# sssxyd/cpp-paddle-ocr

Hardware: AMD Instinct MI355X
Metric: images/sec end-to-end (det+cls+rec) at 960x960 (higher is better)
Workload: dtype f32

## Files before the change

cpp-paddle-ocr_amd/binding.py:

```python
import ctypes as C
import os

import numpy as np

HERE = os.path.dirname(os.path.abspath(__file__))
ROOT = os.path.dirname(HERE)
LIB_PATH = os.environ.get("OCR_LIB_PATH") or os.path.join(HERE, "lib", "libocr_hip.so")
MODELS = os.path.join(ROOT, "models")

_lib = None


class OcrError(RuntimeError):
    pass


class ocr_img(C.Structure):
    _fields_ = [("data", C.c_void_p), ("rows", C.c_int), ("cols", C.c_int), ("row_stride", C.c_size_t)]


class ocr_det_cfg(C.Structure):
    _fields_ = [("model_dir", C.c_char_p), ("device_id", C.c_int), ("limit_type", C.c_char_p),
                ("limit_side_len", C.c_int), ("det_db_thresh", C.c_double), ("det_db_box_thresh", C.c_double),
                ("det_db_unclip_ratio", C.c_double), ("det_db_score_mode", C.c_char_p), ("use_dilation", C.c_int),
# ... 800 lines not shown
class ocr_char(C.Structure):
    _fields_ = [("step", C.c_int32), ("nsteps", C.c_int32), ("prob", C.c_float), ("quad", C.c_int32 * 8)]


EXPORTS += ["ocr_pipe_cfg_default", "ocr_pipe_create", "ocr_pipe_destroy", "ocr_pipe_run", "ocr_pipe_run_chars", "ocr_pipe_run_device",
            "ocr_pipe_stage", "ocr_pipe_slot_probs", "ocr_pipe_run_staged", "ocr_pipe_run_device_on", "ocr_pipe_run_staged_on", "ocr_pipe_stage_jpeg", "ocr_jpeg_decode", "ocr_jpeg_time",
            "ocr_pipe_stage_jpeg_frames", "ocr_jpeg_decode_frame", "ocr_jpeg_time_frame", "ocr_pipe_slot_image",
            "ocr_png_decode", "ocr_png_time", "ocr_png_time_batch", "ocr_pipe_stage_coded",
            "ocr_raw_decode", "ocr_raw_time", "ocr_raw_time_batch", "ocr_pipe_stage_frames",
            "ocr_tiff_decode", "ocr_tiff_time", "ocr_tiff_time_batch", "ocr_pipe_stage_batch",
            "ocr_webp_decode", "ocr_webp_time", "ocr_webp_time_batch", "ocr_vp8_decode", "ocr_vp8_time", "ocr_vp8_time_batch", "ocr_j2k_decode", "ocr_j2k_time", "ocr_j2k_time_batch",
            "ocr_j2k_tier1", "ocr_j2k_decode_coded", "ocr_j2k_time_coded", "ocr_j2k_time_coded_batch",
            "ocr_tiff_expand", "ocr_tiff_decode_coded", "ocr_tiff_time_coded", "ocr_tiff_time_coded_batch",
            "ocr_tiff_inflate", "ocr_tiff_decode_deflate", "ocr_tiff_time_deflate", "ocr_tiff_time_deflate_batch",
            "ocr_pipe_label", "ocr_pipe_det_shape", "ocr_pipe_stats", "ocr_pipe_timing", "ocr_pipe_timing_filter", "ocr_pipe_timing_report", "ocr_dev_alloc",
            "ocr_dev_free", "ocr_dev_upload", "ocr_dev_download", "ocr_dev_sync", "ocr_dev_copy_time", "ocr_rotate_crop", "ocr_rotate_crop_shape", "ocr_rotate180_rois"]


def _pipe_protos(L):
    if getattr(L, "_pipe_protos_done", False):
        return
    _stage_protos(L)
    vp, ip = C.c_void_p, C.POINTER(C.c_int)
    L.ocr_pipe_cfg_default.argtypes = [C.POINTER(ocr_pipe_cfg)]
    L.ocr_pipe_create.argtypes = [C.POINTER(ocr_pipe_cfg), C.POINTER(vp)]
    L.ocr_pipe_destroy.argtypes = [vp]
    L.ocr_pipe_run.argtypes = [vp, C.POINTER(ocr_img), C.c_int, vp, C.c_int, vp, vp, vp, C.c_int, C.POINTER(C.c_double)]
    L.ocr_pipe_run_chars.argtypes = [vp, C.POINTER(ocr_img), C.c_int, vp, C.c_int, vp, vp, vp, C.c_int, vp, C.POINTER(C.c_double)]
    L.ocr_pipe_run_device.argtypes = [vp, vp, C.c_int, C.c_int, C.c_int, vp, vp, C.c_int, vp, vp, vp, C.c_int,
                                      C.POINTER(C.c_double)]
    L.ocr_pipe_stage.argtypes = [vp, C.c_int, C.POINTER(ocr_img), C.c_int]
# ... 473 lines not shown
            maps = [np.ascontiguousarray(p, dtype=np.float32) for p in probs]
            for i, m in enumerate(maps):
                arr[i] = m.ctypes.data
            check(lib().ocr_pipe_slot_probs(self.h, slot, arr, n))

    def stage_dev_probs(self, slot, imgs, dev_probs):
        n = len(imgs)
        self._staged_n = getattr(self, "_staged_n", {})
        check(lib().ocr_pipe_stage(self.h, slot, _imgs(imgs), n))
        self._staged_n[slot] = n
        arr = (C.c_void_p * n)()
        for i, d in enumerate(dev_probs):
            arr[i] = d.ptr.value
        check(lib().ocr_pipe_slot_probs(self.h, slot, arr, n))

    def stats(self):
        out = (C.c_longlong * 3)()
        check(lib().ocr_pipe_stats(self.h, out))
        return dict(runs=int(out[0]), binds=int(out[1]), graph_replays=int(out[2]))

    def run_staged(self, slot, collect=True):
        count = self._staged_n[slot]
        words, ids = self._bufs(count)
        off = np.zeros(count, np.int32)
        nw = np.zeros(count, np.int32)
        check(lib().ocr_pipe_run_staged(self.h, slot, words, self._cap_words, off.ctypes.data, nw.ctypes.data, ids.ctypes.data,
                                        self._cap_ids, self.times))
        return self._collect(count, words, ids, off, nw) if collect else int(nw.sum())

    def run_device(self, dev_imgs, rows, cols, count, dev_prob=None, collect=True):
# ... 67 lines not shown
```

cpp-paddle-ocr_amd/csrc/capi_net.hip:

```cpp
#include <cstdio>
#include <atomic>
#include <cstring>
#include <mutex>
#include <vector>

#include "capi_common.h"
#include "plans_embedded.inc"

__attribute__((constructor)) static void ocr_runtime_env_defaults() { setenv("GPU_MAX_HW_QUEUES", "16", 0); }

namespace ocr {

const RtOptions& rt_options() {
  static RtOptions o;
  static std::once_flag once;
  std::call_once(once, [] {
    auto off = [](const char* n) { const char* e = getenv(n); return e && e[0] == '0'; };
    auto num = [](const char* n, long def) { const char* e = getenv(n); return e && *e ? atol(e) : def; };
    o.fuse = !off("OCR_FUSE");
    o.fuse_gap_min = num("OCR_FUSE_GAP_MIN", 64 * 1024);
    o.conv_small_nt = !off("OCR_CONV_SMALL_NT");
    o.conv_mt2 = !off("OCR_CONV_MT2");
    if (const char* e = getenv("OCR_CONV_MT2")) o.conv_mt2_force = e[0] == 'f';
    o.conv_c24 = !off("OCR_CONV_C24");
    { const char* e = getenv("OCR_DW_LDS"); o.dw_lds = !(e && e[0] == '0'); }
    { const char* e = getenv("OCR_DWPW2"); o.dwpw2 = !(e && e[0] == '0'); }
    { const char* e = getenv("OCR_XDW"); o.xdw = !(e && e[0] == '0'); }
    { const char* e = getenv("OCR_MFMA_X16"); o.mfma_x16 = !(e && e[0] == '0'); }
    { const char* e = getenv("OCR_ATTN_LINE"); o.attn_line = !(e && e[0] == '0'); }
    o.dwpw_items = (int)num("OCR_DWPW_ITEMS", 32);
    o.dwpw_force_upw = (int)num("OCR_DWPW_FORCE_UPW", 0);
    if (const char* e = getenv("OCR_DWPW_T4")) o.dwpw_t4_thin = e[0] == 't';
    o.trace_slice = (int)num("OCR_TRACE_SLICE", 0);
  });
  return o;
}
static std::mutex g_refuse_mu;
static std::string g_refuse;
static std::atomic<bool> g_refuse_on{false};
std::string rt_refuse_launch() {
  if (!g_refuse_on.load(std::memory_order_acquire)) return std::string();
  std::lock_guard<std::mutex> lk(g_refuse_mu);
  return g_refuse;
}
void rt_set_refuse_launch(const char* substr) {
  std::lock_guard<std::mutex> lk(g_refuse_mu);
  g_refuse = substr ? substr : "";
  g_refuse_on.store(!g_refuse.empty(), std::memory_order_release);
// ... 417 lines not shown
```

cpp-paddle-ocr_amd/csrc/pipe.hip:

```cpp
#include <algorithm>
#include <array>
#include <chrono>
#include <cstring>
#include <functional>
#include <map>
#include <memory>
#include <thread>

#include "capi_common.h"
#include "crop.h"
#include "frame_kinds.h"
#include "stages.h"

using namespace ocr;

namespace {
double now_ms() {
  return std::chrono::duration<double, std::milli>(std::chrono::steady_clock::now().time_since_epoch()).count();
}
}

using CharLists = std::vector<std::vector<ocr_char>>;
static int emit(const std::vector<std::vector<ocr_word>>& W, const std::vector<std::vector<int32_t>>& I, const std::vector<int>& order,
                ocr_word* words, int cap_words, int* word_off, int* nwords, int32_t* ids, int cap_ids, const CharLists* C = nullptr,
// ... 87 lines not shown
    return OCR_OK;
  }

  bool timing_on = false;
  std::string timing_filter;
  int add_det_extra(std::string& err) {
    std::unique_ptr<DetStage> d(new DetStage());
    int code = 0;
    if (!d->create(det_cfg, err, code)) return code ? code : OCR_ERR_DEVICE;
    d->net().set_timing_filter(timing_filter);
    d->net().enable_timing(timing_on);
    det_extra.push_back(std::move(d));
    return OCR_OK;
  }

  int run_images(uint8_t* base, const std::vector<StageSlot::Img>& imgs, const std::vector<StageSlot::Group>& groups, const float* probs,
                 std::vector<std::vector<ocr_word>>& out_words, std::vector<std::vector<int32_t>>& out_ids, double times[3], std::string& err,
                 CharLists* out_chars = nullptr) {
    const int count = (int)imgs.size();
    boxes.resize((size_t)count * kCap * 8);
    nbox.assign(count, 0);
    double t0 = now_ms();
    auto run_group = [&](DetStage& d, const StageSlot::Group& g, std::string& e) {
      const size_t row = (size_t)g.cols * 3, img_bytes = row * g.rows;
      return d.run_device(base + g.off, img_bytes, row, g.rows, g.cols, g.count, boxes.data() + (size_t)g.first * kCap * 8, kCap,
                          nbox.data() + g.first, nullptr, e, probs ? probs + g.prob_off : nullptr);
    };
    const int lanes = (int)std::min<size_t>((size_t)det_lanes, groups.size());
    if (groups.size() > 1 && det_ragged) {
      std::vector<DetStage::MixedGroup> mg(groups.size());
      std::vector<size_t> gpx(groups.size());
      for (size_t gi = 0; gi < groups.size(); ++gi) {
        const auto& g = groups[gi];
// ... 62 lines not shown
        for (int l = 0; l < np; ++l)
          if (rcs[l]) { err = errs[l]; return rcs[l]; }
        if (g_stream_sync(src.stream()) != hipSuccess) { err = "det stream sync failed"; return OCR_ERR_DEVICE; }
        src.collect_timings();
      }
    } else if (lanes <= 1) {
      for (const auto& g : groups) {
        int rc = run_group(det, g, err);
        if (rc) return rc;
      }
    } else {
      while ((int)det_extra.size() < lanes - 1) {
        int rc = add_det_extra(err);
        if (rc) return rc;
      }
      if (g_stream_sync(det.stream()) != hipSuccess) { err = "det stream sync failed"; return OCR_ERR_DEVICE; }
      std::vector<int> rcs(lanes, OCR_OK);
      std::vector<std::string> errs(lanes);
      auto lane_fn = [&](int l) {
        DetStage& d = l == 0 ? det : *det_extra[l - 1];
        for (size_t gi = l; gi < groups.size(); gi += lanes) {
          rcs[l] = run_group(d, groups[gi], errs[l]);
          if (rcs[l]) return;
        }
      };
      std::vector<std::thread> th;
      for (int l = 1; l < lanes; ++l) th.emplace_back(lane_fn, l);
      lane_fn(0);
      for (auto& t : th) t.join();
      for (int l = 0; l < lanes; ++l)
        if (rcs[l]) { err = errs[l]; return rcs[l]; }
// ... 25 lines not shown
          lines.push_back(LineSrc{base + imgs[i].off, row, ix0, iy0, ix1 - ix0, iy1 - iy0});
        }
      }
      seg.push_back((int)lines.size());
    }
    out_words.assign(count, {});
    out_ids.assign(count, {});
    if (out_chars) out_chars->assign(count, {});
    if (lines.empty()) return OCR_OK;
    std::vector<int> labels;
    if (cls) {
      labels.resize(lines.size());
      std::vector<float> scores(lines.size());
      int rc = cls->run_lines(lines, labels.data(), scores.data(), err);
      if (rc) return rc;
      std::vector<RotDesc> rd;
      for (size_t k = 0; k < lines.size(); ++k)
        if (labels[k] == 1) rd.push_back(RotDesc{const_cast<uint8_t*>(lines[k].img), lines[k].stride, lines[k].x, lines[k].y, lines[k].w, lines[k].h});
      int rrc = rotate180_in_order(rd, rot_desc, rot_seg, cls->stream(), err);
      if (rrc) return rrc;
      if (g_stream_sync(cls->stream()) != hipSuccess) { err = "cls stream sync failed"; return OCR_ERR_DEVICE; }
    }
    double t2 = now_ms();
    times[1] += t2 - t1;
    const int max_len = 256;
    std::vector<int32_t> ids(lines.size() * max_len);
    std::vector<int> lens(lines.size());
    std::vector<float> scores(lines.size());
    std::vector<int32_t> csteps, cnsteps, geom;
    std::vector<float> cprobs;
    int rc;
    if (out_chars) {
      csteps.resize(ids.size()); cnsteps.resize(ids.size()); cprobs.resize(ids.size()); geom.resize(lines.size() * 3);
      RecStage::CharOut co;
      co.steps = csteps.data(); co.nsteps = cnsteps.data(); co.probs = cprobs.data(); co.geom = geom.data();
      rc = rec.run_lines_chars(lines, seg, ids.data(), max_len, lens.data(), scores.data(), co, err);
// ... 11 lines not shown
        w.confidence = scores[k];
        out_ids[i].insert(out_ids[i].end(), ids.begin() + (size_t)k * max_len, ids.begin() + (size_t)k * max_len + lens[k]);
        out_words[i].push_back(w);
        if (out_chars)
          for (int j = 0; j < lens[k]; ++j) {
            const size_t q = (size_t)k * max_len + j;
            ocr_char ch;
            ch.step = csteps[q]; ch.nsteps = cnsteps[q]; ch.prob = cprobs[q];
            const LineSrc& L = lines[k];
            char_quad(ch.step, ch.nsteps, geom[3 * k], geom[3 * k + 1], geom[3 * k + 2], L.w, L.h, !labels.empty() && labels[k] == 1,
                      crop_mode == OCR_CROP_ROTATE ? &line_plan[k] : nullptr, L.x, L.y, imgs[i].rows, imgs[i].cols, ch.quad);
            (*out_chars)[i].push_back(ch);
          }
      }
    }
    return OCR_OK;
  }

  int rotate_crops(const uint8_t* base, const std::vector<StageSlot::Img>& imgs, std::vector<LineSrc>& lines, std::vector<int>& seg,
                   std::vector<int>& line_box, std::string& err) {
    std::vector<WarpDesc> wd;
    std::vector<size_t> off;
    size_t total = 0;
    int max_px = 0;
    for (int i = 0; i < (int)imgs.size(); ++i) {
      const int rows = imgs[i].rows, cols = imgs[i].cols;
      const size_t row = (size_t)cols * 3;
      for (int j = 0; j < nbox[i]; ++j) {
        CropPlan p;
        if (!plan_rotate_crop(rows, cols, &boxes[((size_t)i * kCap + j) * 8], p)) continue;
// ... 25 lines not shown
    if (g_stream_sync(det.stream()) != hipSuccess) { err = "crop kernel failed"; return OCR_ERR_DEVICE; }
    return OCR_OK;
  }
};

struct ocr_pipe {
  PipeWorker w0;
  std::vector<std::unique_ptr<PipeWorker>> extra;
  int phases = 2;
  int parts_per_chain = 1;
  int device = 0;
  StageSlot slots[2];
  hipStream_t copy_stream = nullptr;
  FrameScratch frame_scratch;
  DevBuf<uint8_t> work;
  DevBuf<uint8_t> work_chain[4];
  PipeWorker* worker(int c) { return c == 0 ? &w0 : (c >= 1 && c <= (int)extra.size() ? extra[c - 1].get() : nullptr); }

  ~ocr_pipe() { if (copy_stream) (void)hipStreamDestroy(copy_stream); }

  int layout(StageSlot& S, int count, const std::function<void(int, int&, int&)>& size_of, std::string& err) {
    if (!copy_stream && hipStreamCreateWithFlags(&copy_stream, hipStreamNonBlocking) != hipSuccess) { err = "hipStreamCreate failed"; return OCR_ERR_DEVICE; }
    if (!S.ready && hipEventCreateWithFlags(&S.ready, hipEventDisableTiming) != hipSuccess) { err = "hipEventCreate failed"; return OCR_ERR_DEVICE; }
    if (S.staged && hipEventSynchronize(S.ready) != hipSuccess) { err = "staging event failed"; return OCR_ERR_DEVICE; }
    S.staged = false;
    std::vector<int> order(count), rows(count), cols(count);
    for (int i = 0; i < count; ++i) { order[i] = i; size_of(i, rows[i], cols[i]); }
    std::stable_sort(order.begin(), order.end(), [&](int a, int b) { return rows[a] != rows[b] ? rows[a] < rows[b] : cols[a] < cols[b]; });
    const std::vector<StageSlot::Img> before = S.imgs;
    S.imgs.clear();
// ... 72 lines not shown
    if (!S.staged || count != (int)S.imgs.size()) { err = "stage the slot's images first (same count)"; return OCR_ERR_ARG; }
    if (!S.probs.ensure(S.prob_floats + 64, err)) return OCR_ERR_DEVICE;
    for (int k = 0; k < count; ++k) {
      const size_t n = (k + 1 < count ? S.imgs[k + 1].prob_off : S.prob_floats) - S.imgs[k].prob_off;
      const hipError_t e = hipMemcpyAsync(S.probs.p + S.imgs[k].prob_off, probs[S.imgs[k].orig], n * sizeof(float), hipMemcpyDefault, copy_stream);
      if (e != hipSuccess) {
        err = std::string("probability map upload failed: ") + hipGetErrorString(e);
        return OCR_ERR_DEVICE;
      }
    }
    if (hipEventRecord(S.ready, copy_stream) != hipSuccess) { err = "hipEventRecord failed"; return OCR_ERR_DEVICE; }
    S.has_probs = true;
    return OCR_OK;
  }

  int run_images(uint8_t* base, const std::vector<StageSlot::Img>& imgs, const std::vector<StageSlot::Group>& groups, const float* probs,
                 std::vector<std::vector<ocr_word>>& out_words, std::vector<std::vector<int32_t>>& out_ids, double times[3], std::string& err,
                 CharLists* out_chars = nullptr) {
    const int count = (int)imgs.size();
    const int nchains = (int)std::min<size_t>(1 + extra.size(), (size_t)count);
    if (nchains < 2) return w0.run_images(base, imgs, groups, probs, out_words, out_ids, times, err, out_chars);
    const int K = (int)std::min<size_t>((size_t)nchains * parts_per_chain, (size_t)count);
    std::vector<std::vector<StageSlot::Img>> pi(K);
    std::vector<std::vector<StageSlot::Group>> pg(K);
    std::vector<std::vector<int>> gidx(K);
    std::vector<size_t> load(K, 0);
    auto give = [&](int p, const StageSlot::Group& g, int first, int n) {
      int rh = 0, rw = 0;
      { float a, b; DetStage::resize_shape(g.rows, g.cols, w0.det.cfg().limit_type, w0.det.cfg().limit_side_len, rh, rw, a, b); }
      StageSlot::Group ng = g;
      ng.first = (int)pi[p].size();
      ng.count = n;
      ng.off = g.off + (size_t)first * g.rows * g.cols * 3;
      ng.prob_off = g.prob_off + (size_t)first * rh * rw;
      pg[p].push_back(ng);
      for (int k = 0; k < n; ++k) { pi[p].push_back(imgs[g.first + first + k]); gidx[p].push_back(g.first + first + k); }
// ... 3 lines not shown
    for (const auto& g : groups) total += (size_t)g.count * g.rows * g.cols;
    const size_t share = (total + K - 1) / K;
    for (const auto& g : groups) {
      const size_t px = (size_t)g.rows * g.cols;
      int first = 0;
      while (first < g.count) {
        const int p = (int)(std::min_element(load.begin(), load.end()) - load.begin());
        const int left = g.count - first;
        const size_t room = share > load[p] ? share - load[p] : 0;
        int n = left;
        if ((size_t)left * px > room + px / 2) n = (int)std::min<size_t>(left, std::max<size_t>(1, (room + px / 2) / px));
        give(p, g, first, n);
        first += n;
      }
    }
    if (g_stream_sync(w0.det.stream()) != hipSuccess) { err = "det stream sync failed"; return OCR_ERR_DEVICE; }
    std::vector<std::vector<std::vector<ocr_word>>> W(K);
    std::vector<std::vector<std::vector<int32_t>>> I(K);
    std::vector<CharLists> Ch(K);
    std::vector<std::array<double, 3>> t(K, std::array<double, 3>{0, 0, 0});
    std::vector<int> rc(K, OCR_OK);
    std::vector<std::string> errs(K);
    auto chain = [&](int c) {
      PipeWorker& w = c == 0 ? w0 : *extra[c - 1];
      for (int p = c; p < K; p += nchains) {
        if (pi[p].empty()) continue;
        rc[p] = w.run_images(base, pi[p], pg[p], probs, W[p], I[p], t[p].data(), errs[p], out_chars ? &Ch[p] : nullptr);
        if (rc[p]) return;
      }
    };
    std::vector<std::thread> th;
    for (int c = 1; c < nchains; ++c) th.emplace_back([&, c]() { (void)rt_set_device(device); chain(c); });
    chain(0);
    for (auto& x : th) x.join();
    for (int p = 0; p < K; ++p)
      if (rc[p]) { err = errs[p]; return rc[p]; }
    out_words.assign(count, {});
    out_ids.assign(count, {});
    if (out_chars) out_chars->assign(count, {});
    for (int p = 0; p < K; ++p)
      for (size_t k = 0; k < gidx[p].size(); ++k) {
        out_words[gidx[p][k]] = std::move(W[p][k]);
// ... 11 lines not shown
    }
    return OCR_OK;
  }

  int run_slot(int si, ocr_word* words, int cap_words, int* word_off, int* nwords, int32_t* ids, int cap_ids, double times[3], int chain = -1,
               ocr_char* chars = nullptr) {
    StageSlot& S = slots[si];
    if (!S.staged || S.imgs.empty()) return fail(OCR_ERR_ARG, "nothing staged in this slot");
    std::string err;
    PipeWorker* one = chain >= 0 ? worker(chain) : nullptr;
    if (chain >= 0 && !one) return fail(OCR_ERR_ARG, "no such chain (0 <= chain < phases)");
    PipeWorker& first = one ? *one : w0;
    DevBuf<uint8_t>& clone = one ? work_chain[chain] : work;
    if (hipStreamWaitEvent(first.det.stream(), S.ready, 0) != hipSuccess) return fail(OCR_ERR_DEVICE, "hipStreamWaitEvent failed");
    if (!clone.ensure(S.bytes + 256, err)) return fail(OCR_ERR_DEVICE, err);
    if (hipMemcpyAsync(clone.p, S.dev.p, S.bytes, hipMemcpyDeviceToDevice, first.det.stream()) != hipSuccess) return fail(OCR_ERR_DEVICE, "clone failed");
    double t[3] = {0, 0, 0};
    std::vector<std::vector<ocr_word>> W;
    std::vector<std::vector<int32_t>> I;
    CharLists C;
    CharLists* pc = chars ? &C : nullptr;
    const int rc = one ? one->run_images(clone.p, S.imgs, S.groups, S.has_probs ? S.probs.p : nullptr, W, I, t, err, pc)
                       : run_images(clone.p, S.imgs, S.groups, S.has_probs ? S.probs.p : nullptr, W, I, t, err, pc);
    if (rc) return fail(rc, err);
    if (times) { times[0] = t[0]; times[1] = t[1]; times[2] = t[2]; }
    const int count = (int)S.imgs.size();
    std::vector<int> order(count);
    for (int k = 0; k < count; ++k) order[S.imgs[k].orig] = k;
    return emit(W, I, order, words, cap_words, word_off, nwords, ids, cap_ids, pc, chars);
  }
};

static int emit(const std::vector<std::vector<ocr_word>>& W, const std::vector<std::vector<int32_t>>& I, const std::vector<int>& order,
                ocr_word* words, int cap_words, int* word_off, int* nwords, int32_t* ids, int cap_ids, const CharLists* C, ocr_char* chars) {
  int wo = 0, io = 0;
  for (size_t i = 0; i < order.size(); ++i) {
    const auto& w = W[order[i]];
    const auto& d = I[order[i]];
// ... 80 lines not shown
static int pipe_run_device(ocr_pipe* h, int chain, const void* dev_bgr, int rows, int cols, int count, const float* dev_prob, ocr_word* words,
                           int cap_words, int* word_off, int* nwords, int32_t* ids, int cap_ids, double times[3]) {
  if (!h || !dev_bgr || rows <= 0 || cols <= 0 || count < 1 || !words || !word_off || !nwords || !ids)
    return fail(OCR_ERR_ARG, "bad argument");
  CAPI_HIP(rt_set_device(h->device));
  PipeWorker* one = chain >= 0 ? h->worker(chain) : nullptr;
  if (chain >= 0 && !one) return fail(OCR_ERR_ARG, "no such chain (0 <= chain < phases)");
  PipeWorker& first = one ? *one : h->w0;
  DevBuf<uint8_t>& clone = one ? h->work_chain[chain] : h->work;
  double t[3] = {0, 0, 0};
  std::vector<std::vector<ocr_word>> W;
  std::vector<std::vector<int32_t>> I;
  std::string err;
  const size_t img_bytes = (size_t)rows * cols * 3, bytes = img_bytes * count;
  if (!clone.ensure(bytes + 256, err)) return fail(OCR_ERR_DEVICE, err);
  CAPI_HIP(hipMemcpyAsync(clone.p, dev_bgr, bytes, hipMemcpyDeviceToDevice, first.det.stream()));
  std::vector<StageSlot::Img> imgs(count);
  for (int i = 0; i < count; ++i) imgs[i] = {rows, cols, i, img_bytes * i, 0};
  const std::vector<StageSlot::Group> groups = {{rows, cols, 0, count, 0, 0}};
  const int rc = one ? one->run_images(clone.p, imgs, groups, dev_prob, W, I, t, err) : h->run_images(clone.p, imgs, groups, dev_prob, W, I, t, err);
  if (rc) return fail(rc, err);
  if (times) { times[0] = t[0]; times[1] = t[1]; times[2] = t[2]; }
  std::vector<int> order(count);
  for (int i = 0; i < count; ++i) order[i] = i;
  return emit(W, I, order, words, cap_words, word_off, nwords, ids, cap_ids);
}
int ocr_pipe_run_device(ocr_pipe* h, const void* dev_bgr, int rows, int cols, int count, const float* dev_prob, ocr_word* words,
                        int cap_words, int* word_off, int* nwords, int32_t* ids, int cap_ids, double times[3]) {
  return pipe_run_device(h, -1, dev_bgr, rows, cols, count, dev_prob, words, cap_words, word_off, nwords, ids, cap_ids, times);
}
int ocr_pipe_run_device_on(ocr_pipe* h, int chain, const void* dev_bgr, int rows, int cols, int count, const float* dev_prob,
                           ocr_word* words, int cap_words, int* word_off, int* nwords, int32_t* ids, int cap_ids, double times[3]) {
  if (chain < 0) return fail(OCR_ERR_ARG, "no such chain (0 <= chain < phases)");
  return pipe_run_device(h, chain, dev_bgr, rows, cols, count, dev_prob, words, cap_words, word_off, nwords, ids, cap_ids, times);
}
// ... 290 lines not shown
  DevBuf<int> dseg;
  if (!dimg.ensure(row * rows, err)) return fail(OCR_ERR_DEVICE, err);
  std::vector<RotDesc> rd(n);
  for (int k = 0; k < n; ++k) {
    const int32_t* r = rects + 4 * k;
    if (r[0] < 0 || r[1] < 0 || r[2] < 1 || r[3] < 1 || r[0] + r[2] > cols || r[1] + r[3] > rows) return fail(OCR_ERR_ARG, "rectangle outside the image");
    rd[k] = RotDesc{dimg.p, row, r[0], r[1], r[2], r[3]};
  }
  CAPI_HIP(g_memcpy2d(dimg.p, row, bgr, stride, row, rows, hipMemcpyHostToDevice));
  const int rc = rotate180_in_order(rd, ddesc, dseg, 0, err);
  if (rc) return fail(rc, err);
  CAPI_HIP(g_memcpy2d(bgr, stride, dimg.p, row, row, rows, hipMemcpyDeviceToHost));
  return OCR_OK;
}

int ocr_dev_alloc(void** p, size_t bytes) {
  if (!p) return fail(OCR_ERR_ARG, "null argument");
  CAPI_HIP(g_malloc(p, bytes));
  return OCR_OK;
}
int ocr_dev_free(void* p) { CAPI_HIP(g_free(p)); return OCR_OK; }
int ocr_dev_upload(void* dst, const void* src, size_t bytes) { CAPI_HIP(g_memcpy(dst, src, bytes, hipMemcpyHostToDevice)); return OCR_OK; }
int ocr_dev_download(void* dst, const void* src, size_t bytes) { CAPI_HIP(g_memcpy(dst, src, bytes, hipMemcpyDeviceToHost)); return OCR_OK; }
int ocr_dev_sync(void) { CAPI_HIP(hipDeviceSynchronize()); return OCR_OK; }

}
```

cpp-paddle-ocr_amd/csrc/rt_options.h:

```cpp
#pragma once
#include <string>

namespace ocr {

struct RtOptions {
  bool fuse = true;
  long fuse_gap_min = 65536;
  bool conv_small_nt = true;
  bool conv_mt2 = true;
  bool conv_mt2_force = false;
  bool conv_c24 = true;
  bool attn_line = true;
  bool mfma_x16 = true;
  bool dw_lds = true;
  bool xdw = true;
  bool dwpw2 = true;
  int dwpw_items = 32;
  int dwpw_force_upw = 0;
  bool dwpw_t4_thin = false;
  int trace_slice = 0;
};
const RtOptions& rt_options();

std::string rt_refuse_launch();
void rt_set_refuse_launch(const char* substr);

}
```

cpp-paddle-ocr_amd/csrc/stages.h:

```cpp
#pragma once
#include <hip/hip_runtime.h>

#include <memory>
#include <string>
#include <vector>

#include "../../include/ocr_hip.h"
#include "kernels_post.h"
#include "kernels_pre.h"
#include "net.h"
#include "srv_net.h"

namespace ocr {

template <class T>
struct DevBuf {
  T* p = nullptr;
  size_t cap = 0;
  ~DevBuf() { if (p) (void)g_free(p); }
  bool ensure(size_t n, std::string& err) {
    if (n <= cap) return true;
    if (p) (void)g_free(p);
    p = nullptr;
    cap = 0;
// ... 116 lines not shown
                float* scores, std::string& err, const CharOut* co = nullptr);
  int run_chars(const ocr_img* imgs, int n, int32_t* ids, int max_len, int* lens, float* scores, const CharOut& co, double times[3],
                std::string& err);
  int run_lines_chars(const std::vector<LineSrc>& lines, const std::vector<int>& seg, int32_t* ids, int max_len, int* lens,
                      float* scores, const CharOut& co, std::string& err) {
    return run_lines(lines, seg, ids, max_len, lens, scores, err, &co);
  }
  int logits_row(int index, int step, float* out, size_t cap_floats, std::string& err);
  bool want_taps = true;
  int max_lines_per_launch = 4096;
  const std::vector<std::string>& labels() const { return labels_; }
  hipStream_t stream() const { return stream_; }
  Net& net() { return net_; }
  SrvNet* srv() { return srv_.get(); }
  std::vector<int> tap_T, tap_off;
  std::vector<int> tap_amax;
  std::vector<float> tap_pmax;

 private:
  RecConfig cfg_;
  Net net_;
  std::unique_ptr<SrvNet> srv_;
  hipStream_t stream_ = nullptr;
  StageTimer timer_;
  std::vector<std::string> labels_;
  DevBuf<float> lut_, pmax_, scores_, x_;
  DevBuf<int> amax_, ids_, lens_;
  DevBuf<uint8_t> staging_;
  DevBuf<LineDesc> descs_;
  DevBuf<int> csteps_, cnsteps_, alt_ids_;
// ... 42 lines not shown
```

cpp-paddle-ocr_amd/csrc/stages.hip:

```cpp
#include "stages.h"

#include <algorithm>
#include <array>
#include <cmath>
#include <cstring>
#include <fstream>
#include <map>

#include "capi_common.h"

namespace ocr {

#define ST_HIP(expr)                                                              \
  do {                                                                            \
    hipError_t _e = (expr);                                                       \
    if (_e != hipSuccess) {                                                       \
      err = std::string(#expr) + ": " + hipGetErrorString(_e);                    \
      return OCR_ERR_DEVICE;                                                      \
    }                                                                             \
  } while (0)

bool StageTimer::init(std::string& err) {
  for (int i = 0; i < 4; ++i)
    if (hipEventCreate(&ev[i]) != hipSuccess) { err = "hipEventCreate failed"; return false; }
// ... 673 lines not shown
  auto mobile_logits = [&](Net::HeadLogits& hl, const Slot& sl, bool ragged) -> int {
    if (topk <= 0) return OCR_OK;
    if (!net_.head_logits(hl, err)) return OCR_ERR_DEVICE;
    if (hl.C != C) { err = "dictionary size does not match the CTC head"; return OCR_ERR_MODEL; }
    if (ragged)
      for (int j = 0; j < sl.count; ++j)
        if ((int)hl.row0.size() != sl.count + 1 || hl.row0[j] != d[sl.first + j].step0) { err = "ragged logits rows do not match the step table"; return OCR_ERR_DEVICE; }
    return OCR_OK;
  };
  ST_HIP(hipMemcpyAsync(descs_.p, d.data(), (size_t)ni * sizeof(LineDesc), hipMemcpyHostToDevice, stream_));
  for (Slot& sl : slots) {
    if (!srv_) net_.set_head_outputs(nullptr, amax_.p + sl.step_off, pmax_.p + sl.step_off);
    if (srv_) {
      const int Wt = items[sl.first].tensor_w;
      launch_line_pre(descs_.p + sl.first, sl.count, imgH, Wt, lut_.p, false, x_.p, stream_);
      if (!srv_->run(x_.p, sl.count, imgH, Wt, stream_, err)) return OCR_ERR_DEVICE;
      const SrvTensor& ot = srv_->tensor(srv_->output_tid());
      if (ot.h != 1) { err = "rec_img_h does not reduce to a single row"; return OCR_ERR_ARG; }
      if (ot.c != (int)labels_.size()) { err = "dictionary size does not match the CTC head"; return OCR_ERR_MODEL; }
      sl.T = ot.w;
      if (sl.T > Wt / 4 + 8) { err = "rec step buffer too small"; return OCR_ERR_CAPACITY; }
      if (srv_->ctc_partials())
        srv::launch_ctc_reduce((const float*)srv_->tensor_ptr(srv_->output_tid()), (long)sl.count * sl.T, srv_->ctc_slots(), srv_->ctc_step(),
                               amax_.p + sl.step_off, pmax_.p + sl.step_off, stream_);
      else
        srv::launch_argmax_softmax((const float*)srv_->tensor_ptr(srv_->output_tid()), (long)sl.count * sl.T, ot.c, ot.cs, amax_.p + sl.step_off,
                                   pmax_.p + sl.step_off, srv_->half(), stream_);
      if (co) {
        const int rc = collapse(sl, nullptr, sl.T, (const float*)srv_->tensor_ptr(srv_->output_tid()), ot.cs);
        if (rc) return rc;
      } else
      launch_ctc(amax_.p + sl.step_off, pmax_.p + sl.step_off, sl.count, sl.T, max_len, ids_.p + (size_t)sl.first * max_len,
                 lens_.p + sl.first, scores_.p + sl.first, stream_);
    } else if (sl.ragged) {
      widths.resize(sl.count);
      long pix = 0;
      for (int j = 0; j < sl.count; ++j) { widths[j] = items[sl.first + j].tensor_w; pix += (long)imgH * widths[j]; }
      launch_line_pre_ragged(descs_.p + sl.first, sl.count, pix, imgH, lut_.p, x_.p, stream_);
      if (!net_.run_ragged(x_.p, imgH, widths.data(), sl.count, stream_, err)) return OCR_ERR_DEVICE;
      if (co) {
        Net::HeadLogits hl;
        int rc = mobile_logits(hl, sl, true);
        if (!rc) rc = collapse(sl, descs_.p + sl.first, 0, hl.ptr, hl.pitch);
        if (rc) return rc;
      } else
      launch_ctc_ragged(amax_.p + sl.step_off, pmax_.p + sl.step_off, descs_.p + sl.first, sl.count, max_len,
                        ids_.p + (size_t)sl.first * max_len, lens_.p + sl.first, scores_.p + sl.first, stream_);
    } else {
      const int Wt = items[sl.first].tensor_w;
      launch_line_pre(descs_.p + sl.first, sl.count, imgH, Wt, lut_.p, false, x_.p, stream_);
      if (!net_.run(x_.p, sl.count, imgH, Wt, stream_, err)) return OCR_ERR_DEVICE;
      const TensorDesc& ot = net_.tensor(net_.output_tid());
      if (ot.h != 1) { err = "rec_img_h does not reduce to a single row"; return OCR_ERR_ARG; }
      if (ot.c != (int)labels_.size()) { err = "dictionary size does not match the CTC head"; return OCR_ERR_MODEL; }
      sl.T = ot.w;
      if (sl.T > Wt / 4 + 8) { err = "rec step buffer too small"; return OCR_ERR_CAPACITY; }
      if (co) {
        Net::HeadLogits hl;
        int rc = mobile_logits(hl, sl, false);
        if (!rc) rc = collapse(sl, nullptr, sl.T, hl.ptr, hl.pitch);
        if (rc) return rc;
      } else
      launch_ctc(amax_.p + sl.step_off, pmax_.p + sl.step_off, sl.count, sl.T, max_len, ids_.p + (size_t)sl.first * max_len,
                 lens_.p + sl.first, scores_.p + sl.first, stream_);
    }
// ... 131 lines not shown
```

include/ocr_hip.h:

```cpp
#ifndef OCR_HIP_H_
#define OCR_HIP_H_

#include <stddef.h>
#include <stdint.h>

#ifdef __cplusplus
extern "C" {
#endif

#define OCR_OK 0
#define OCR_ERR_ARG (-1)
#define OCR_ERR_MODEL (-2)
#define OCR_ERR_DEVICE (-3)
#define OCR_ERR_CAPACITY (-4)

const char* ocr_last_error(void);
int ocr_rt_init(int device_id);
int ocr_rt_device_count(void);
int ocr_rt_set_wait_mode(int mode);
int ocr_rt_get_wait_mode(void);

typedef struct ocr_img {
  const uint8_t* data;
  int rows, cols;
// ... 325 lines not shown
} ocr_coded_frame;
int ocr_pipe_stage_batch(ocr_pipe* h, int slot, const ocr_coded_frame* frames, int count);
const char* ocr_pipe_label(ocr_pipe* h, int id);
int ocr_pipe_det_shape(ocr_pipe* h, int rows, int cols, int* net_rows, int* net_cols);
int ocr_pipe_stats(ocr_pipe* h, long long out[3]);
int ocr_pipe_timing(ocr_pipe* h, int enable);
int ocr_pipe_timing_filter(ocr_pipe* h, const char* substr);
int ocr_pipe_timing_report(ocr_pipe* h, char* buf, size_t cap);

int ocr_rotate_crop(const uint8_t* bgr, int rows, int cols, size_t row_stride, const int32_t* boxes, int n, uint8_t* out,
                    size_t out_cap, size_t* out_off, int* out_rows, int* out_cols);
int ocr_rotate_crop_shape(int rows, int cols, const int32_t* box, int* out_rows, int* out_cols);

int ocr_rotate180_rois(uint8_t* bgr, int rows, int cols, size_t row_stride, const int32_t* rects, int n);

int ocr_dev_alloc(void** p, size_t bytes);
int ocr_dev_free(void* p);
int ocr_dev_upload(void* dst, const void* src, size_t bytes);
int ocr_dev_download(void* dst, const void* src, size_t bytes);
int ocr_dev_sync(void);
int ocr_dev_copy_time(void* dst, const void* src, size_t bytes, int iters, double* ms);

typedef struct ocr_net ocr_net;
int ocr_net_create(const char* kind, const char* model_dir, const char* weights, int device_id, ocr_net** out);
int ocr_net_create_precision(const char* kind, const char* model_dir, const char* weights, int device_id, const char* precision,
                             ocr_net** out);
void ocr_net_destroy(ocr_net* h);
int ocr_net_forward(ocr_net* h, const float* x, int N, int H, int W, int keep_all);
int ocr_net_forward_ragged(ocr_net* h, const float* x, int N, int H, const int* widths, int keep_all);
int ocr_net_forward_ragged_images(ocr_net* h, const float* x, int N, const int* heights, const int* widths, int keep_all);
// ... 75 lines not shown
```

Measured before the change: 1234.

## Clone staged images lazily, only those whose crops the classifier rotates

Stops copying the whole staged image batch into a work buffer before detection. Only images that contain a line classified as upside-down are copied, with adjacent images merged into one copy, and their lines are redirected to the copy before the in-place 180-degree rotation. The source buffer is no longer modified. When lazy cloning is on, the det stream sync before the lanes is skipped because no clone copy has to finish, and the cls stream sync is skipped when nothing is rotated. The risk is an ordering hazard between the reduced syncs and the det and rec streams. A self-test entry point and a flag to turn the behaviour off are also added.

```diff
diff --git a/cpp-paddle-ocr_amd/binding.py b/cpp-paddle-ocr_amd/binding.py
--- a/cpp-paddle-ocr_amd/binding.py
+++ b/cpp-paddle-ocr_amd/binding.py
@@ -838,7 +838,8 @@
             "ocr_tiff_expand", "ocr_tiff_decode_coded", "ocr_tiff_time_coded", "ocr_tiff_time_coded_batch",
             "ocr_tiff_inflate", "ocr_tiff_decode_deflate", "ocr_tiff_time_deflate", "ocr_tiff_time_deflate_batch",
             "ocr_pipe_label", "ocr_pipe_det_shape", "ocr_pipe_stats", "ocr_pipe_timing", "ocr_pipe_timing_filter", "ocr_pipe_timing_report", "ocr_dev_alloc",
-            "ocr_dev_free", "ocr_dev_upload", "ocr_dev_download", "ocr_dev_sync", "ocr_dev_copy_time", "ocr_rotate_crop", "ocr_rotate_crop_shape", "ocr_rotate180_rois"]
+            "ocr_dev_free", "ocr_dev_upload", "ocr_dev_download", "ocr_dev_sync", "ocr_dev_copy_time", "ocr_rotate_crop", "ocr_rotate_crop_shape", "ocr_rotate180_rois",
+            "ocr_selftest_pipe_lazy_clone", "ocr_selftest_pipe_turns"]
 
 
 def _pipe_protos(L):
@@ -1342,6 +1343,30 @@
             arr[i] = d.ptr.value
         check(lib().ocr_pipe_slot_probs(self.h, slot, arr, n))
 
+    def set_lazy_clone(self, on):
+        L = lib()
+        L.ocr_selftest_pipe_lazy_clone.argtypes = [C.c_void_p, C.c_int]
+        check(L.ocr_selftest_pipe_lazy_clone(self.h, int(bool(on))))
+
+    def selftest_turns(self, imgs, rects, labels, owner):
+        imgs = np.ascontiguousarray(imgs, dtype=np.uint8)
+        assert imgs.ndim == 4 and imgs.shape[3] == 3
+        rects = np.ascontiguousarray(rects, dtype=np.int32).reshape(-1, 4)
+        labels = np.ascontiguousarray(labels, dtype=np.int32)
+        owner = np.ascontiguousarray(owner, dtype=np.int32)
+        assert len(rects) == len(labels) == len(owner)
+        cap = len(rects) * 48 * max(320, max(48 * int(w) // max(1, int(h)) + 48 for _, _, w, h in rects)) * 3
+        x = np.zeros(cap, np.float32)
+        after = np.zeros_like(imgs)
+        nfl, ncp = C.c_size_t(0), C.c_int(0)
+        L = lib()
+        L.ocr_selftest_pipe_turns.argtypes = [C.c_void_p, C.c_void_p, C.c_int, C.c_int, C.c_int, C.c_void_p, C.c_void_p, C.c_void_p, C.c_int,
+                                              C.c_void_p, C.c_void_p, C.c_size_t, C.POINTER(C.c_size_t), C.POINTER(C.c_int)]
+        check(L.ocr_selftest_pipe_turns(self.h, imgs.ctypes.data, imgs.shape[1], imgs.shape[2], imgs.shape[0], rects.ctypes.data,
+                                        labels.ctypes.data, owner.ctypes.data, len(rects), after.ctypes.data, x.ctypes.data, cap,
+                                        C.byref(nfl), C.byref(ncp)))
+        return x[:nfl.value].copy(), after, int(ncp.value)
+
     def stats(self):
         out = (C.c_longlong * 3)()
         check(lib().ocr_pipe_stats(self.h, out))
diff --git a/cpp-paddle-ocr_amd/csrc/capi_net.hip b/cpp-paddle-ocr_amd/csrc/capi_net.hip
--- a/cpp-paddle-ocr_amd/csrc/capi_net.hip
+++ b/cpp-paddle-ocr_amd/csrc/capi_net.hip
@@ -32,6 +32,7 @@
     o.dwpw_force_upw = (int)num("OCR_DWPW_FORCE_UPW", 0);
     if (const char* e = getenv("OCR_DWPW_T4")) o.dwpw_t4_thin = e[0] == 't';
     o.trace_slice = (int)num("OCR_TRACE_SLICE", 0);
+    o.lazy_clone = !off("OCR_LAZY_CLONE");
   });
   return o;
 }
diff --git a/cpp-paddle-ocr_amd/csrc/pipe.hip b/cpp-paddle-ocr_amd/csrc/pipe.hip
--- a/cpp-paddle-ocr_amd/csrc/pipe.hip
+++ b/cpp-paddle-ocr_amd/csrc/pipe.hip
@@ -125,9 +125,9 @@
     return OCR_OK;
   }
 
-  int run_images(uint8_t* base, const std::vector<StageSlot::Img>& imgs, const std::vector<StageSlot::Group>& groups, const float* probs,
-                 std::vector<std::vector<ocr_word>>& out_words, std::vector<std::vector<int32_t>>& out_ids, double times[3], std::string& err,
-                 CharLists* out_chars = nullptr) {
+  int run_images(const uint8_t* base, uint8_t* clone, bool lead, const std::vector<StageSlot::Img>& imgs,
+                 const std::vector<StageSlot::Group>& groups, const float* probs, std::vector<std::vector<ocr_word>>& out_words,
+                 std::vector<std::vector<int32_t>>& out_ids, double times[3], std::string& err, CharLists* out_chars = nullptr) {
     const int count = (int)imgs.size();
     boxes.resize((size_t)count * kCap * 8);
     nbox.assign(count, 0);
@@ -220,7 +220,7 @@
         int rc = add_det_extra(err);
         if (rc) return rc;
       }
-      if (g_stream_sync(det.stream()) != hipSuccess) { err = "det stream sync failed"; return OCR_ERR_DEVICE; }
+      if (lead && g_stream_sync(det.stream()) != hipSuccess) { err = "det stream sync failed"; return OCR_ERR_DEVICE; }
       std::vector<int> rcs(lanes, OCR_OK);
       std::vector<std::string> errs(lanes);
       auto lane_fn = [&](int l) {
@@ -276,12 +276,8 @@
       std::vector<float> scores(lines.size());
       int rc = cls->run_lines(lines, labels.data(), scores.data(), err);
       if (rc) return rc;
-      std::vector<RotDesc> rd;
-      for (size_t k = 0; k < lines.size(); ++k)
-        if (labels[k] == 1) rd.push_back(RotDesc{const_cast<uint8_t*>(lines[k].img), lines[k].stride, lines[k].x, lines[k].y, lines[k].w, lines[k].h});
-      int rrc = rotate180_in_order(rd, rot_desc, rot_seg, cls->stream(), err);
-      if (rrc) return rrc;
-      if (g_stream_sync(cls->stream()) != hipSuccess) { err = "cls stream sync failed"; return OCR_ERR_DEVICE; }
+      rc = turn_crops(base, clone, imgs, seg, labels, lines, nullptr, err);
+      if (rc) return rc;
     }
     double t2 = now_ms();
     times[1] += t2 - t1;
@@ -323,6 +319,40 @@
           }
       }
     }
+    return OCR_OK;
+  }
+
+  int turn_crops(const uint8_t* base, uint8_t* clone, const std::vector<StageSlot::Img>& imgs, const std::vector<int>& seg,
+                 const std::vector<int>& labels, std::vector<LineSrc>& lines, int* ncopied, std::string& err) {
+    if (clone && crop_mode != OCR_CROP_ROTATE) {
+      size_t run_off = 0, run_len = 0;
+      auto flush = [&]() {
+        const bool ok = run_len == 0 || hipMemcpyAsync(clone + run_off, base + run_off, run_len, hipMemcpyDeviceToDevice, cls->stream()) == hipSuccess;
+        run_len = 0;
+        return ok;
+      };
+      for (int i = 0; i < (int)imgs.size(); ++i) {
+        bool turned = false;
+        for (int k = seg[i]; k < seg[i + 1] && !turned; ++k) turned = labels[k] == 1;
+        if (!turned) continue;
+        const size_t bytes = (size_t)imgs[i].rows * imgs[i].cols * 3;
+        if (run_len && run_off + run_len == imgs[i].off) run_len += bytes;
+        else {
+          if (!flush()) { err = "clone failed"; return OCR_ERR_DEVICE; }
+          run_off = imgs[i].off;
+          run_len = bytes;
+        }
+        for (int k = seg[i]; k < seg[i + 1]; ++k) lines[k].img = clone + imgs[i].off;
+        if (ncopied) ++*ncopied;
+      }
+      if (!flush()) { err = "clone failed"; return OCR_ERR_DEVICE; }
+    }
+    std::vector<RotDesc> rd;
+    for (size_t k = 0; k < lines.size(); ++k)
+      if (labels[k] == 1) rd.push_back(RotDesc{const_cast<uint8_t*>(lines[k].img), lines[k].stride, lines[k].x, lines[k].y, lines[k].w, lines[k].h});
+    const int rrc = rotate180_in_order(rd, rot_desc, rot_seg, cls->stream(), err);
+    if (rrc) return rrc;
+    if (!rd.empty() && g_stream_sync(cls->stream()) != hipSuccess) { err = "cls stream sync failed"; return OCR_ERR_DEVICE; }
     return OCR_OK;
   }
 
@@ -378,6 +408,7 @@
   hipStream_t copy_stream = nullptr;
   FrameScratch frame_scratch;
   DevBuf<uint8_t> work;
+  bool lazy_clone = rt_options().lazy_clone;
   DevBuf<uint8_t> work_chain[4];
   PipeWorker* worker(int c) { return c == 0 ? &w0 : (c >= 1 && c <= (int)extra.size() ? extra[c - 1].get() : nullptr); }
 
@@ -480,12 +511,12 @@
     return OCR_OK;
   }
 
-  int run_images(uint8_t* base, const std::vector<StageSlot::Img>& imgs, const std::vector<StageSlot::Group>& groups, const float* probs,
-                 std::vector<std::vector<ocr_word>>& out_words, std::vector<std::vector<int32_t>>& out_ids, double times[3], std::string& err,
-                 CharLists* out_chars = nullptr) {
+  int run_images(const uint8_t* base, uint8_t* clone, bool lead, const std::vector<StageSlot::Img>& imgs,
+                 const std::vector<StageSlot::Group>& groups, const float* probs, std::vector<std::vector<ocr_word>>& out_words,
+                 std::vector<std::vector<int32_t>>& out_ids, double times[3], std::string& err, CharLists* out_chars = nullptr) {
     const int count = (int)imgs.size();
     const int nchains = (int)std::min<size_t>(1 + extra.size(), (size_t)count);
-    if (nchains < 2) return w0.run_images(base, imgs, groups, probs, out_words, out_ids, times, err, out_chars);
+    if (nchains < 2) return w0.run_images(base, clone, lead, imgs, groups, probs, out_words, out_ids, times, err, out_chars);
     const int K = (int)std::min<size_t>((size_t)nchains * parts_per_chain, (size_t)count);
     std::vector<std::vector<StageSlot::Img>> pi(K);
     std::vector<std::vector<StageSlot::Group>> pg(K);
@@ -519,7 +550,7 @@
         first += n;
       }
     }
-    if (g_stream_sync(w0.det.stream()) != hipSuccess) { err = "det stream sync failed"; return OCR_ERR_DEVICE; }
+    if (lead && g_stream_sync(w0.det.stream()) != hipSuccess) { err = "det stream sync failed"; return OCR_ERR_DEVICE; }
     std::vector<std::vector<std::vector<ocr_word>>> W(K);
     std::vector<std::vector<std::vector<int32_t>>> I(K);
     std::vector<CharLists> Ch(K);
@@ -530,7 +561,7 @@
       PipeWorker& w = c == 0 ? w0 : *extra[c - 1];
       for (int p = c; p < K; p += nchains) {
         if (pi[p].empty()) continue;
-        rc[p] = w.run_images(base, pi[p], pg[p], probs, W[p], I[p], t[p].data(), errs[p], out_chars ? &Ch[p] : nullptr);
+        rc[p] = w.run_images(base, clone, false, pi[p], pg[p], probs, W[p], I[p], t[p].data(), errs[p], out_chars ? &Ch[p] : nullptr);
         if (rc[p]) return;
       }
     };
@@ -572,14 +603,17 @@
     DevBuf<uint8_t>& clone = one ? work_chain[chain] : work;
     if (hipStreamWaitEvent(first.det.stream(), S.ready, 0) != hipSuccess) return fail(OCR_ERR_DEVICE, "hipStreamWaitEvent failed");
     if (!clone.ensure(S.bytes + 256, err)) return fail(OCR_ERR_DEVICE, err);
-    if (hipMemcpyAsync(clone.p, S.dev.p, S.bytes, hipMemcpyDeviceToDevice, first.det.stream()) != hipSuccess) return fail(OCR_ERR_DEVICE, "clone failed");
+    if (!lazy_clone && hipMemcpyAsync(clone.p, S.dev.p, S.bytes, hipMemcpyDeviceToDevice, first.det.stream()) != hipSuccess)
+      return fail(OCR_ERR_DEVICE, "clone failed");
+    const uint8_t* base = lazy_clone ? S.dev.p : clone.p;
+    uint8_t* lazy = lazy_clone ? clone.p : nullptr;
     double t[3] = {0, 0, 0};
     std::vector<std::vector<ocr_word>> W;
     std::vector<std::vector<int32_t>> I;
     CharLists C;
     CharLists* pc = chars ? &C : nullptr;
-    const int rc = one ? one->run_images(clone.p, S.imgs, S.groups, S.has_probs ? S.probs.p : nullptr, W, I, t, err, pc)
-                       : run_images(clone.p, S.imgs, S.groups, S.has_probs ? S.probs.p : nullptr, W, I, t, err, pc);
+    const int rc = one ? one->run_images(base, lazy, true, S.imgs, S.groups, S.has_probs ? S.probs.p : nullptr, W, I, t, err, pc)
+                       : run_images(base, lazy, true, S.imgs, S.groups, S.has_probs ? S.probs.p : nullptr, W, I, t, err, pc);
     if (rc) return fail(rc, err);
     if (times) { times[0] = t[0]; times[1] = t[1]; times[2] = t[2]; }
     const int count = (int)S.imgs.size();
@@ -690,11 +724,15 @@
   std::string err;
   const size_t img_bytes = (size_t)rows * cols * 3, bytes = img_bytes * count;
   if (!clone.ensure(bytes + 256, err)) return fail(OCR_ERR_DEVICE, err);
-  CAPI_HIP(hipMemcpyAsync(clone.p, dev_bgr, bytes, hipMemcpyDeviceToDevice, first.det.stream()));
+  const bool lazy = h->lazy_clone;
+  if (!lazy) CAPI_HIP(hipMemcpyAsync(clone.p, dev_bgr, bytes, hipMemcpyDeviceToDevice, first.det.stream()));
+  const uint8_t* base = lazy ? (const uint8_t*)dev_bgr : clone.p;
+  uint8_t* lazy_to = lazy ? clone.p : nullptr;
   std::vector<StageSlot::Img> imgs(count);
   for (int i = 0; i < count; ++i) imgs[i] = {rows, cols, i, img_bytes * i, 0};
   const std::vector<StageSlot::Group> groups = {{rows, cols, 0, count, 0, 0}};
-  const int rc = one ? one->run_images(clone.p, imgs, groups, dev_prob, W, I, t, err) : h->run_images(clone.p, imgs, groups, dev_prob, W, I, t, err);
+  const int rc = one ? one->run_images(base, lazy_to, !lazy, imgs, groups, dev_prob, W, I, t, err)
+                     : h->run_images(base, lazy_to, !lazy, imgs, groups, dev_prob, W, I, t, err);
   if (rc) return fail(rc, err);
   if (times) { times[0] = t[0]; times[1] = t[1]; times[2] = t[2]; }
   std::vector<int> order(count);
@@ -1015,6 +1053,56 @@
   return OCR_OK;
 }
 
+int ocr_selftest_pipe_lazy_clone(ocr_pipe* h, int on) {
+  if (!h) return fail(OCR_ERR_ARG, "null argument");
+  h->lazy_clone = on != 0;
+  return OCR_OK;
+}
+
+int ocr_selftest_pipe_turns(ocr_pipe* h, const uint8_t* bgr, int rows, int cols, int count, const int32_t* rects, const int32_t* labels,
+                            const int32_t* owner, int n, uint8_t* bgr_after, float* x, size_t cap_floats, size_t* nfloats, int* ncopied) {
+  if (!h || !bgr || !rects || !labels || !owner || !bgr_after || !x || !nfloats || !ncopied) return fail(OCR_ERR_ARG, "null argument");
+  if (rows < 1 || cols < 1 || rows > 4096 || cols > 4096 || count < 1 || count > 16 || n < 1 || n > 256) return fail(OCR_ERR_ARG, "size out of range");
+  if (!h->w0.cls) return fail(OCR_ERR_ARG, "the pipeline has no classifier");
+  if (h->w0.crop_mode != OCR_CROP_BOUNDING_RECT) return fail(OCR_ERR_ARG, "crop_mode is not OCR_CROP_BOUNDING_RECT");
+  CAPI_HIP(rt_set_device(h->device));
+  const size_t row = (size_t)cols * 3, img_bytes = row * rows, bytes = img_bytes * count;
+  std::vector<StageSlot::Img> imgs(count);
+  for (int i = 0; i < count; ++i) imgs[i] = {rows, cols, i, img_bytes * i, 0};
+  std::string err;
+  DevBuf<uint8_t> src;
+  if (!src.ensure(bytes, err) || !h->work.ensure(bytes + 256, err)) return fail(OCR_ERR_DEVICE, err);
+  CAPI_HIP(g_memcpy(src.p, bgr, bytes, hipMemcpyHostToDevice));
+  const bool lazy = h->lazy_clone;
+  if (!lazy) CAPI_HIP(g_memcpy(h->work.p, src.p, bytes, hipMemcpyDeviceToDevice));
+  CAPI_HIP(g_stream_sync(nullptr));
+  const uint8_t* base = lazy ? src.p : h->work.p;
+  std::vector<LineSrc> lines(n);
+  std::vector<int> seg(1, 0), lab(labels, labels + n);
+  for (int k = 0; k < n; ++k) {
+    const int32_t* r = rects + 4 * k;
+    if (r[0] < 0 || r[1] < 0 || r[2] < 1 || r[3] < 1 || r[0] > cols - r[2] || r[1] > rows - r[3]) return fail(OCR_ERR_ARG, "rectangle outside the image");
+    if (owner[k] < 0 || owner[k] >= count || (k && owner[k] < owner[k - 1])) return fail(OCR_ERR_ARG, "owner is not an ascending list of image indices");
+    while ((int)seg.size() <= owner[k]) seg.push_back(k);
+    lines[k] = LineSrc{base + imgs[owner[k]].off, row, r[0], r[1], r[2], r[3]};
+  }
+  while ((int)seg.size() <= count) seg.push_back(n);
+  *ncopied = 0;
+  int rc = h->w0.turn_crops(base, lazy ? h->work.p : nullptr, imgs, seg, lab, lines, ncopied, err);
+  if (rc) return fail(rc, err);
+  const int max_len = 256;
+  std::vector<int32_t> ids((size_t)n * max_len);
+  std::vector<int> lens(n);
+  std::vector<float> scores(n);
+  rc = h->w0.rec.run_lines(lines, seg, ids.data(), max_len, lens.data(), scores.data(), err);
+  if (rc) return fail(rc, err);
+  *nfloats = h->w0.rec.tap_x_floats;
+  if (*nfloats > cap_floats) return fail(OCR_ERR_CAPACITY, "input tensor larger than the buffer");
+  CAPI_HIP(g_memcpy(x, h->w0.rec.input(), *nfloats * sizeof(float), hipMemcpyDeviceToHost));
+  CAPI_HIP(g_memcpy(bgr_after, src.p, bytes, hipMemcpyDeviceToHost));
+  return OCR_OK;
+}
+
 int ocr_dev_alloc(void** p, size_t bytes) {
   if (!p) return fail(OCR_ERR_ARG, "null argument");
   CAPI_HIP(g_malloc(p, bytes));
diff --git a/cpp-paddle-ocr_amd/csrc/rt_options.h b/cpp-paddle-ocr_amd/csrc/rt_options.h
--- a/cpp-paddle-ocr_amd/csrc/rt_options.h
+++ b/cpp-paddle-ocr_amd/csrc/rt_options.h
@@ -19,6 +19,7 @@
   int dwpw_force_upw = 0;
   bool dwpw_t4_thin = false;
   int trace_slice = 0;
+  bool lazy_clone = true;
 };
 const RtOptions& rt_options();
 
diff --git a/cpp-paddle-ocr_amd/csrc/stages.h b/cpp-paddle-ocr_amd/csrc/stages.h
--- a/cpp-paddle-ocr_amd/csrc/stages.h
+++ b/cpp-paddle-ocr_amd/csrc/stages.h
@@ -154,6 +154,8 @@
   Net& net() { return net_; }
   SrvNet* srv() { return srv_.get(); }
   std::vector<int> tap_T, tap_off;
+  size_t tap_x_floats = 0;
+  const float* input() const { return x_.p; }
   std::vector<int> tap_amax;
   std::vector<float> tap_pmax;
 
diff --git a/cpp-paddle-ocr_amd/csrc/stages.hip b/cpp-paddle-ocr_amd/csrc/stages.hip
--- a/cpp-paddle-ocr_amd/csrc/stages.hip
+++ b/cpp-paddle-ocr_amd/csrc/stages.hip
@@ -711,6 +711,7 @@
     if (srv_) {
       const int Wt = items[sl.first].tensor_w;
       launch_line_pre(descs_.p + sl.first, sl.count, imgH, Wt, lut_.p, false, x_.p, stream_);
+      tap_x_floats = (size_t)sl.count * imgH * Wt * 3;
       if (!srv_->run(x_.p, sl.count, imgH, Wt, stream_, err)) return OCR_ERR_DEVICE;
       const SrvTensor& ot = srv_->tensor(srv_->output_tid());
       if (ot.h != 1) { err = "rec_img_h does not reduce to a single row"; return OCR_ERR_ARG; }
@@ -734,6 +735,7 @@
       long pix = 0;
       for (int j = 0; j < sl.count; ++j) { widths[j] = items[sl.first + j].tensor_w; pix += (long)imgH * widths[j]; }
       launch_line_pre_ragged(descs_.p + sl.first, sl.count, pix, imgH, lut_.p, x_.p, stream_);
+      tap_x_floats = (size_t)pix * 3;
       if (!net_.run_ragged(x_.p, imgH, widths.data(), sl.count, stream_, err)) return OCR_ERR_DEVICE;
       if (co) {
         Net::HeadLogits hl;
@@ -746,6 +748,7 @@
     } else {
       const int Wt = items[sl.first].tensor_w;
       launch_line_pre(descs_.p + sl.first, sl.count, imgH, Wt, lut_.p, false, x_.p, stream_);
+      tap_x_floats = (size_t)sl.count * imgH * Wt * 3;
       if (!net_.run(x_.p, sl.count, imgH, Wt, stream_, err)) return OCR_ERR_DEVICE;
       const TensorDesc& ot = net_.tensor(net_.output_tid());
       if (ot.h != 1) { err = "rec_img_h does not reduce to a single row"; return OCR_ERR_ARG; }
diff --git a/include/ocr_hip.h b/include/ocr_hip.h
--- a/include/ocr_hip.h
+++ b/include/ocr_hip.h
@@ -363,6 +363,10 @@
 
 int ocr_rotate180_rois(uint8_t* bgr, int rows, int cols, size_t row_stride, const int32_t* rects, int n);
 
+int ocr_selftest_pipe_lazy_clone(ocr_pipe* h, int on);
+int ocr_selftest_pipe_turns(ocr_pipe* h, const uint8_t* bgr, int rows, int cols, int count, const int32_t* rects, const int32_t* labels,
+                            const int32_t* owner, int n, uint8_t* bgr_after, float* x, size_t cap_floats, size_t* nfloats, int* ncopied);
+
 int ocr_dev_alloc(void** p, size_t bytes);
 int ocr_dev_free(void* p);
 int ocr_dev_upload(void* dst, const void* src, size_t bytes);
```

Result: no change. 1235 (median of 5 runs) (+0.0%).
